# iagostorch/VVC-MIP-GPU

Measured on AMD Instinct MI355X. Metric: 1080p frames/sec, full MIP mode search over all CU sizes; 1/2/4/8 GPU, higher is better.
Workload: dtype int16x2/int32

## Files before the change

vvc-mip-gpu_amd/csrc/mip_kernels.h:

```cpp
#pragma once
#include <hip/hip_runtime.h>
#include <stdint.h>

#include "mipgpu.h"

namespace mipgpu {

struct Job {
  uint32_t cost;
  uint8_t lx, ly;
  uint16_t cu;
};
struct WaveTask {
  uint8_t cls;
  uint8_t ncu;
  uint8_t q0, q1;
  uint32_t cu0;
};

constexpr int kNumClasses = 29;
constexpr int kNumBaseClasses = 17;
constexpr int kClassW[kNumClasses] = {64, 32, 32, 16, 32, 8, 16, 16, 8, 32, 4, 16, 4, 8, 8, 4, 4, 32, 16, 16, 8,
                                      4, 4, 4, 8, 8, 8, 32, 16};
constexpr int kClassH[kNumClasses] = {64, 32, 16, 32, 8, 32, 16, 8, 16, 4, 32, 4, 16, 8, 4, 8, 4, 8, 16, 8, 16,
// ... 25 lines not shown
  uint8_t *best_mode;
  int32_t *best_cost;
  uint32_t *split_acc;
  const uint16_t *dfill;
  const int *dfill_begin;
  int32_t *sad;
  int32_t *satd;
  const WaveTask *tasks;
  const Job *jobs;
  const int *list_begin;
  const uint32_t *fill;
  const int *fill_begin;
  const uint8_t *ctu_var;
  const uint4 *tables;
  int width, height;
  int ctu_cols, nctus;
  int ctu0, nrange;
  int slices;
  uint32_t *queue;
  uint32_t nitems;
  const uint32_t *order;
  uint32_t nframes;
  uint32_t chunks;
  uint64_t *wave_clock;
  uint32_t *status;
  uint32_t *const *frame_status;
  int check_refs;
  uint32_t nonempty;
};
constexpr int kStatusOrig = 0, kStatusRefs = 1, kStatusWords = 4;
constexpr uint32_t kAbove10Bits = 0xfc00fc00u;
constexpr int kClockSlots = 128;
constexpr int kQueueChunks = 8;
constexpr int kQueueWords = 16;
constexpr int kMaxCtuVariants = 255;

constexpr float kAccInitS2 = 0.5f - 1024.0f;
constexpr int kWeightRows = 768, kWeightRowOffS1 = 384, kWeightRowOffS0 = 512;
constexpr int kCtabRows = 384 + 4;
constexpr int kTableBytes = kWeightRows * 16 + kCtabRows * 4;

struct FixupCu {
  uint32_t ctu;
  uint16_t cu;
  uint8_t shape;
  uint8_t pad;
// ... 72 lines not shown
```

vvc-mip-gpu_amd/csrc/mip_search.hip:

```cpp
#include <algorithm>
#include <cstdlib>
#include <type_traits>
#include <utility>

#include <hip/hip_ext.h>

#ifndef MIP_FOUR_WAVE_TWIN
#define MIP_FOUR_WAVE_TWIN 0
#endif
#if MIP_FOUR_WAVE_TWIN
#define launch_search launch_search_four
#define search_resident_groups search_resident_groups_four
#define search_lds_bytes search_lds_bytes_four
#endif

#include "mip_kernels.h"
#include "mip_tables.h"

namespace mipgpu {
namespace {

typedef short __attribute__((ext_vector_type(2))) s2;
typedef unsigned short __attribute__((ext_vector_type(2))) u2;
typedef _Float16 __attribute__((ext_vector_type(2))) h2;
// ... 86 lines not shown
__device__ __forceinline__ void static_for_impl(F &f, std::integer_sequence<int, I...>) {
  (f(std::integral_constant<int, I>{}), ...);
}
template <int N, class F>
__device__ __forceinline__ void static_for(F &&f) {
  static_for_impl(f, std::make_integer_sequence<int, N>{});
}

template <int O>
__device__ __forceinline__ u2 pk_mad_c(u2 a, u2 c) {
  if constexpr (O == 1) {
    return a + c;
  } else {
    u2 d;
    asm("v_pk_mad_u16 %0, %1, %2, %3 op_sel_hi:[1,0,1]" : "=v"(d) : "v"(a), "i"(O), "v"(c));
    return d;
  }
}
template <int O, int C>
__device__ __forceinline__ u2 pk_mad_cc(u2 a) {
  u2 d;
  asm("v_pk_mad_u16 %0, %1, %2, %3 op_sel_hi:[1,0,0]" : "=v"(d) : "v"(a), "i"(O), "i"(C));
  return d;
}

__device__ __forceinline__ void wave_lds_sync() {
  __builtin_amdgcn_fence(__ATOMIC_RELEASE, "wavefront");
  __builtin_amdgcn_wave_barrier();
  __builtin_amdgcn_fence(__ATOMIC_ACQUIRE, "wavefront");
}

template <int W, int H, int VP = kClassV[size_class(W, H)]>
struct Geo {
  static constexpr int SID = class_size_id(W, H);
  static constexpr int R = SID == 2 ? 8 : 4;
  static constexpr int RBS = SID == 0 ? 2 : 4;
  static constexpr int NOUT = R * R;
  static constexpr int UH = W / R, UV = H / R;
  static constexpr int LH = ilog2c(UH), LV = ilog2c(UV);
  static constexpr int S = W / 4;
  static constexpr int V = VP;
  static constexpr int SLOTS = 64 / (S * V);
  static constexpr int KV = R / V;
  static constexpr int CROWS = UH != 1 ? (kSpanChunks && 64 / (S * V) * (R * (R + 1) + 1) > kScratchWords ? R / 2 : R)
                               : 64 / (S * V) * (NOUT + 4) <= kScratchWords ? R
                               : !kSpanChunks ? (SID == 2 ? R / 2 : R)
// ... 721 lines not shown
          emit(std::integral_constant<int, w * G::UV + r>{}, prow);
        });
#pragma unroll
        for (int cc = 0; cc < 4; cc++) prev[cc] = next[cc];
      });
    }
    if constexpr (ORIG::TR) {
      acc.t0 = pair_finish_tr(t0, acc.t0);
      acc.t1 = pair_finish_tr(t1, acc.t1);
    } else {
      acc.t0 = pair_finish(t0, acc.t0);
      acc.t1 = pair_finish(t1, acc.t1);
    }
  }
}

struct Ctx {
  const SearchArgs *a;
  const uint16_t *org;
  const uint16_t *ref;
  const uint8_t *w;
  const uint8_t *zero;
  uint8_t *wave;
  int ctu, frame;
  int fx0, fy0;
};

__device__ __forceinline__ uint32_t floor_sat(float f) { return (uint32_t)f; }

template <int W, int H, int V, bool TR>
__device__ __forceinline__ void phase_a(const Ctx &x, int lane, int ncu, int q, int chunk) {
  using G = Geo<W, H, V>;
  const int r = lane & 15, h = lane >> 4;
  const int m0 = TR ? 2 * q - G::MODES : 2 * q;
  constexpr bool HALF = G::CHUNKED && G::SID != 2;
  constexpr bool TR2 = TR && G::SID == 2 && G::CHUNKED && G::CROWS == 2;
  const int jrow = TR2 ? 8 * (r >> 1) + (r & 1) : (G::SID == 2 && TR) ? 8 * (r >> 2) + (r & 3) : r;
  const uint8_t *abase = x.w + ((G::WBASE + (m0 + (h >> 1)) * G::NOUT + jrow) * 8 + 4 * (h & 1)) * 2;
  const bool bsel = (h >> 1) == (r & 1);
  const uint8_t *bbase = bsel ? x.wave + (r >> 1) * kEntryBytes + 8 * ((h & 1) ^ (TR ? 1 : 0)) : x.zero;
  f4 cin;
  if constexpr (G::SID == 2) {
    cin = *reinterpret_cast<const f4 *>(reinterpret_cast<const float *>(x.w + kWeightRows * 16) + 384);
  } else {
    const float *ct = reinterpret_cast<const float *>(x.w + kWeightRows * 16) + (G::WBASE - kWeightRowOffS1);
    cin = *reinterpret_cast<const f4 *>(ct + (m0 + (r & 1)) * G::NOUT + 4 * h);
  }
  constexpr int NCS = (G::SLOTS + 7) / 8;
// ... 112 lines not shown
#define MIP_PIN_SUMS 1
#endif
__device__ __forceinline__ uint32_t pin_sum(uint32_t v) {
#if MIP_PIN_SUMS
  asm volatile("; pin" : "+v"(v));
#endif
  return v;
}

#ifndef MIP_COST_STORE_AUX
#define MIP_COST_STORE_AUX 0
#endif
struct CtuRows {
  __amdgpu_buffer_rsrc_t r;
  __device__ __forceinline__ explicit CtuRows(int32_t *ctu_block) {
    r = __builtin_amdgcn_make_buffer_rsrc(ctu_block, 0, MIP_COSTS_PER_CTU * 4, 0x00020000);
  }
  __device__ __forceinline__ void store(uint32_t cu_ofs, int mq, int v0, int v1) const {
    typedef unsigned int v2u __attribute__((ext_vector_type(2)));
    __builtin_amdgcn_raw_buffer_store_b64((v2u){(unsigned)v0, (unsigned)v1}, r, (int)cu_ofs, mq * 4, MIP_COST_STORE_AUX);
  }
};

__device__ __forceinline__ int opaque(int v) {
  asm volatile("; opaque" : "+v"(v));
  return v;
}

template <bool TR, bool LAT>
struct ViewOf {
  using type = RefTile<LAT>;
  static __device__ __forceinline__ type make(const RefTile<LAT> &r) { return r; }
};
template <bool LAT>
struct ViewOf<true, LAT> {
  using type = RefTileT<LAT>;
  static __device__ __forceinline__ type make(const RefTile<LAT> &r) { return RefTileT<LAT>{r}; }
};

template <int W, int H, int V, bool LAT, bool DEC, bool TR = false>
__device__ __forceinline__ void run_task(const Ctx &x, const RefTile<LAT> &rt_tile, const WaveTask &task, int lane_in) {
  using G = Geo<W, H, V>;
  const typename ViewOf<TR, LAT>::type rt = ViewOf<TR, LAT>::make(rt_tile);
  const int lane = opaque(lane_in);
  const SearchArgs &a = *x.a;
  const int ncu = task.ncu;
  const Job *jobs = a.jobs + task.cu0;
  const int slot = lane / (G::S * G::V), sub = lane % (G::S * G::V);
  const int v = sub / G::S, sx = sub % G::S, x0 = 4 * sx;
  const bool active = slot < ncu;
  const int cs = min(slot, ncu - 1);
  const Job job = jobs[cs];
  const CuPos c = cu_pos<TR>(job, x.fx0, x.fy0, rt);

  if (lane < ncu) {
    const Job jb = jobs[lane];
    const CuPos cj = cu_pos<TR>(jb, x.fx0, x.fy0, rt);
    write_inputs<W, H>(cj, rt, x.wave + lane * kEntryBytes);
  }
  std::conditional_t<TR, OrigRowsT<H>, OrigRows<H>> orig;
  orig.load(x.org, c.lx + x0, c.ly);
  const size_t ctu_row = ((size_t)x.frame * a.nctus + x.ctu) * MIP_COSTS_PER_CTU;
  const uint32_t cu_ofs = (uint32_t)job.cost * 4;
  const CtuRows rows_cost(a.cost ? a.cost + ctu_row : nullptr), rows_sad(a.sad ? a.sad + ctu_row : nullptr),
      rows_satd(a.satd ? a.satd + ctu_row : nullptr);
  const uint32_t *mine = reinterpret_cast<const uint32_t *>(x.wave + kCuTableBytes) + cs * G::PITCH;
  const Red<G::R, G::RP> red{mine, 0};
  s2 top[4];
  {
    const uint2 tv = rt.top4(c.lx + x0, c.ly - 1);
    const int t4[4] = {(int)(tv.x & 0xffff), (int)(tv.x >> 16), (int)(tv.y & 0xffff), (int)(tv.y >> 16)};
#pragma unroll
    for (int cc = 0; cc < 4; cc++) top[cc] = splat(c.top ? t4[cc] : c.padT);
  }
  constexpr int NLV = (G::R + G::S * G::V - 1) / (G::S * G::V);
  uint32_t lvs[G::PAD && G::CHUNKED ? NLV : 1];
  uint32_t *lcol = reinterpret_cast<uint32_t *>(x.wave + kCuTableBytes) + cs * G::PITCH;
  auto write_left = [&](int chunk) {
#pragma unroll
    for (int j = 0; j < NLV; j++) {
      const int k = sub + j * G::S * G::V;
      if (active && k < G::R && k / G::CROWS == chunk) lcol[(k - chunk * G::CROWS) * G::RP] = lvs[j];
    }
  };
  if constexpr (G::PAD && G::CHUNKED) {
// ... 86 lines not shown
      sad0 = sp & 0xffff, sad1 = sp >> 16, satd0 = tp & 0xffff, satd1 = tp >> 16;
    } else {
      acc.flush();
      sad0 = pin_sum(group_sum<GS>(acc.sad0));
      sad1 = pin_sum(group_sum<GS>(acc.sad1));
      satd0 = pin_sum(group_sum<GS>(acc.satd0));
      satd1 = pin_sum(group_sum<GS>(acc.satd1));
      c0 = min(2 * (int)sad0, (int)satd0);
      c1 = min(2 * (int)sad1, (int)satd1);
    }
    if (active && sub == GS - 1) {
      const int mq = TR ? (2 * q < G::MODES ? 2 * q + G::MODES : 2 * q - G::MODES) : 2 * q;
      if constexpr (DEC) {
        best = min(best, min((uint32_t)c0 << 5 | (uint32_t)mq, (uint32_t)c1 << 5 | (uint32_t)(mq + 1)));
      } else {
        rows_cost.store(cu_ofs, mq, c0, c1);
        if (a.sad) rows_sad.store(cu_ofs, mq, (int)sad0, (int)sad1);
        if (a.satd) rows_satd.store(cu_ofs, mq, (int)satd0, (int)satd1);
      }
    }
  }
  if (DEC && active && sub == G::S * G::V - 1) {
    constexpr int kPairs = G::SID == 2 ? 6 : (G::SID == 1 ? 8 : 16);
    const size_t g = ((size_t)x.frame * a.nctus + x.ctu) * MIP_CUS_PER_CTU + job.cu;
    if (task.q0 == 0 && task.q1 == kPairs) {
      if (a.best_mode) a.best_mode[g] = (uint8_t)(best & 31);
      a.best_cost[g] = (int32_t)(best >> 5);
    } else {
      atomicMin((a.split_acc ? a.split_acc : reinterpret_cast<uint32_t *>(a.best_cost)) + g, best);
    }
  }
}

__device__ __forceinline__ uint2 frame_chunk(const uint16_t *frame, int width, int height, int fx, int fy) {
  const int li = fy * width + fx;
  uint2 v = make_uint2(0, 0);
  if (fy >= 0 && fx >= 0 && li < width * height) v = *reinterpret_cast<const uint2 *>(frame + li);
  return v;
}

template <int P>
struct WindowStager {
  static constexpr int RIT = P / 16;
  static constexpr int NMAIN = (65 + RIT - 1) / RIT;
  static constexpr int NHALO = (65 + P - 1) / P;
  static constexpr int N = NMAIN + NHALO;
  static constexpr uint32_t kOut = 0x80000000u;
// ... 26 lines not shown
      if (k == 0 && top) o = p < 16 ? kOut : o;
    } else {
      o = vhalo + (uint32_t)((k - NMAIN) * P) * W2;
      if (left) o = kOut;
      if (k == NMAIN && top) o = p == 0 ? kOut : o;
    }
    typedef unsigned int v2u __attribute__((ext_vector_type(2)));
    const v2u v = __builtin_amdgcn_raw_buffer_load_b64(rsrc, (int)o, 0, 0);
    return make_uint2(v.x, v.y);
  }
  __device__ __forceinline__ void store(uint16_t *dst, int k, uint2 v) const {
    if (k < NMAIN) {
      v.x += bmx;
      v.y += bmy;
      *reinterpret_cast<uint2 *>(dst + (p / 16 + RIT * k) * kPitch + 4 + 4 * (p & 15)) = v;
    } else {
      v.x += bhx;
      v.y += bhy;
      *reinterpret_cast<uint2 *>(dst + (p + P * (k - NMAIN)) * kPitch) = v;
    }
  }
};

#ifndef MIP_FRAME_STATUS
#define MIP_FRAME_STATUS 1
#endif
__device__ __forceinline__ void flag_above_10_bits(uint32_t bits, const SearchArgs &a, int frame, int word) {
  if (bits & kAbove10Bits) (MIP_FRAME_STATUS && a.frame_status ? a.frame_status[frame] : a.status)[word] = 1u;
}

template <int NT>
__device__ __forceinline__ void stage_tile(uint16_t *dst, const uint16_t *frame, int width, int height,
                                           int x0, int y0, const SearchArgs &a, int fidx) {
  const WindowStager<NT> st(frame, width, height, x0, y0, (int)threadIdx.x);
  constexpr int N = WindowStager<NT>::N;
  uint2 v[N];
#pragma unroll
  for (int k = 0; k < N; k++)
    if (st.valid(k)) v[k] = st.load(k);
  uint32_t bits = 0;
#pragma unroll
  for (int k = 0; k < N; k++)
    if (st.valid(k)) {
      bits |= v[k].x | v[k].y;
      st.store(dst, k, v[k]);
    }
  flag_above_10_bits(bits, a, fidx, kStatusOrig);
}

struct ItemPos {
  int frame, ctu, slice, quad, ctu_x, ctu_y, fx0, fy0;
  __device__ __forceinline__ ItemPos(const SearchArgs &a, uint32_t item) {
    const int per_ctu = 4 * a.slices;
    uint32_t base = item;
    if (a.order) {
      base = a.order[item / a.nframes];
      frame = item % a.nframes;
    } else {
      frame = item / (per_ctu * a.nrange);
    }
    const int gx = base % per_ctu;
    ctu = a.ctu0 + (base / per_ctu) % a.nrange;
    slice = gx % a.slices;
    quad = gx / a.slices;
    ctu_x = 128 * (ctu % a.ctu_cols);
    ctu_y = 128 * (ctu / a.ctu_cols);
    fx0 = ctu_x + 64 * (quad & 1);
    fy0 = ctu_y + 64 * (quad >> 1);
  }
};

template <int NT>
__device__ __forceinline__ void stage_lattice(uint16_t *dst, const uint16_t *frame, int width, int height,
                                              int x0, int y0, bool check, const SearchArgs &a, int fidx) {
  constexpr int kChunks = kPitch / 4, NR = 16 * kChunks, NC = 16 * 65;
  constexpr int NRL = (NR + NT - 1) / NT, NCL = (NC + NT - 1) / NT;
  uint2 rv[NRL];
  uint16_t cv[NCL];
#pragma unroll
  for (int k = 0; k < NRL; k++) {
    const int i = min((int)threadIdx.x + NT * k, NR - 1), row = i / kChunks, ch = i - row * kChunks;
    rv[k] = frame_chunk(frame, width, height, x0 - kColOff + 4 * ch, y0 + 4 * row - 1);
  }
#pragma unroll
  for (int k = 0; k < NCL; k++) {
    const int i = min((int)threadIdx.x + NT * k, NC - 1), col = i / 65, yy = i - col * 65;
    const int fy = y0 + yy - 1, fx = x0 + 4 * col - 1, li = fy * width + fx;
    cv[k] = (fy >= 0 && fx >= 0 && li < width * height) ? frame[li] : 0;
  }
  uint32_t bits = 0;
  const bool exempt_last = width % 128 != 0;
  auto frame_col = [&](int fx) { return fx < width ? fx : fx % width; };
#pragma unroll
  for (int k = 0; k < NRL; k++) {
    const int i = min((int)threadIdx.x + NT * k, NR - 1), row = i / kChunks, ch = i - row * kChunks;
    *reinterpret_cast<uint2 *>(dst + row * kLatRowPitch + 4 * ch) = rv[k];
    if (check) {
      const int fx = x0 - kColOff + 4 * ch;
      const bool skip_y = exempt_last && fx >= 0 && frame_col(fx) == width - 4;
      bits |= rv[k].x | (skip_y ? 0u : rv[k].y);
    }
  }
  uint16_t *cols = dst + 16 * kLatRowPitch;
#pragma unroll
  for (int k = 0; k < NCL; k++) {
    const int i = min((int)threadIdx.x + NT * k, NC - 1), col = i / 65, yy = i - col * 65;
    cols[col * kLatColPitch + yy] = cv[k];
    if (check) {
      const int fx = x0 + 4 * col - 1;
      if (!(exempt_last && fx >= 0 && frame_col(fx) == width - 1)) bits |= cv[k];
    }
  }
  if (check) flag_above_10_bits(bits, a, fidx, kStatusRefs);
}

template <bool ALT, bool PF, int NW = kSearchWaves>
constexpr int kOrgTiles = (PF || NW == kWideWaves) && !ALT ? 2 : 1;
constexpr int kCounterWords = 12;

__device__ __forceinline__ uint32_t queue_chunks(const SearchArgs &a) { return gridDim.x < a.chunks ? gridDim.x : a.chunks; }
__device__ __forceinline__ uint32_t chunk_begin(uint32_t nitems, uint32_t c, uint32_t k) {
  return (uint32_t)((uint64_t)nitems * c / k);
}
__device__ __forceinline__ uint32_t take_item(const SearchArgs &a, uint32_t *empty) {
  const uint32_t k = queue_chunks(a), g = blockIdx.x % k;
  for (uint32_t j = *empty; j < k; j++) {
    const uint32_t c = g + j < k ? g + j : g + j - k;
    const uint32_t b = chunk_begin(a.nitems, c, k), n = chunk_begin(a.nitems, c + 1, k) - b;
    const uint32_t i = atomicAdd(a.queue + c, 1u);
    if (i < n) {
      *empty = j;
      return b + i;
    }
  }
  *empty = k;
  return a.nitems;
}
__device__ __forceinline__ bool far_from_end(const SearchArgs &a, uint32_t item) {
  const uint32_t k = queue_chunks(a), g = blockIdx.x % k;
  const uint32_t b = chunk_begin(a.nitems, g, k), e = chunk_begin(a.nitems, g + 1, k);
  return item >= b && item + 3 * (gridDim.x / k) < e;
}
constexpr uint32_t kTakeItem = 0xffffffffu;

template <bool DEC>
__device__ __forceinline__ void fill_unavailable(const SearchArgs &a, int frame, int ctu, int vq, int slice) {
  if (DEC) {
    const size_t gbase = ((size_t)frame * a.nctus + ctu) * MIP_CUS_PER_CTU;
    const int f0 = a.dfill_begin[vq], nf = a.dfill_begin[vq + 1] - f0;
    for (int i = slice * blockDim.x + threadIdx.x; i < nf; i += a.slices * blockDim.x) {
      const size_t g = gbase + a.dfill[f0 + i];
      if (a.best_mode) a.best_mode[g] = 0xff;
      a.best_cost[g] = kUnavailable;
    }
  } else {
    const size_t cbase = ((size_t)frame * a.nctus + ctu) * (MIP_COSTS_PER_CTU / 4);
    const int f0 = a.fill_begin[vq], nf = a.fill_begin[vq + 1] - f0;
    const uint4 un = make_uint4(kUnavailable, kUnavailable, kUnavailable, kUnavailable);
    for (int i = slice * blockDim.x + threadIdx.x; i < nf; i += a.slices * blockDim.x) {
      const size_t o = cbase + a.fill[f0 + i];
      reinterpret_cast<uint4 *>(a.cost)[o] = un;
      if (a.sad) reinterpret_cast<uint4 *>(a.sad)[o] = un;
      if (a.satd) reinterpret_cast<uint4 *>(a.satd)[o] = un;
    }
  }
}

template <bool ALT, bool DEC>
__device__ __forceinline__ void dispatch_task(const Ctx &x, const RefTile<ALT> &rt, const WaveTask &task, int lane) {
  switch (task.cls) {
#define MIP_CASE(idx, W, H)                                                \
  case idx:                                                                \
    static_assert(kClassW[idx] == W && kClassH[idx] == H, "class table");  \
    if constexpr ((MIP_ONLY_CLASS < 0 || MIP_ONLY_CLASS == idx) && !((MIP_SKIP_CLASSES >> idx) & 1)) \
      run_task<W, H, kClassV[idx], ALT, DEC>(x, rt, task, lane);           \
    break;
    MIP_CASE(0, 64, 64) MIP_CASE(1, 32, 32) MIP_CASE(2, 32, 16) MIP_CASE(3, 16, 32)
    MIP_CASE(4, 32, 8) MIP_CASE(5, 8, 32) MIP_CASE(6, 16, 16) MIP_CASE(7, 16, 8)
    MIP_CASE(8, 8, 16) MIP_CASE(9, 32, 4) MIP_CASE(10, 4, 32) MIP_CASE(11, 16, 4)
// ... 4 lines not shown
#undef MIP_CASE
#define MIP_CASE_TR(idx, W, H)                                                    \
  case idx:                                                                       \
    static_assert(kClassW[idx] == W && kClassH[idx] == H && kClassTR[idx], "class table"); \
    if constexpr ((MIP_ONLY_CLASS < 0 || MIP_ONLY_CLASS == idx) && !((MIP_SKIP_CLASSES >> idx) & 1)) \
      run_task<W, H, kClassV[idx], ALT, DEC, true>(x, rt, task, lane);            \
    break;
    MIP_CASE_TR(21, 4, 32) MIP_CASE_TR(22, 4, 16) MIP_CASE_TR(23, 4, 8) MIP_CASE_TR(24, 8, 32)
    MIP_CASE_TR(25, 8, 16) MIP_CASE_TR(26, 8, 16)
#undef MIP_CASE_TR
    default: break;
  }
}

__device__ __forceinline__ void stamp_item_start(uint64_t *clk) {
  clk[kClockSlots - 3] = __builtin_amdgcn_s_memrealtime();
  clk[kClockSlots - 1] = (uint64_t)__builtin_amdgcn_s_getreg((31 << 11) | 4) |
                         (uint64_t)__builtin_amdgcn_s_getreg((31 << 11) | 20) << 32;
}

template <int NT>
__device__ __forceinline__ void stage_tiles2(uint16_t *dst0, const uint16_t *frame0, int x0, int y0, uint16_t *dst1,
                                             const uint16_t *frame1, int x1, int y1, bool b, int width, int height,
                                             const SearchArgs &a, int f0, int f1) {
  const WindowStager<NT> s0(frame0, width, height, x0, y0, (int)threadIdx.x);
  const WindowStager<NT> s1(frame1, width, height, x1, y1, (int)threadIdx.x);
  constexpr int N = WindowStager<NT>::N;
  uint2 v0[N], v1[N];
#pragma unroll
  for (int k = 0; k < N; k++) {
    if (s0.valid(k)) v0[k] = s0.load(k);
    if (b && s1.valid(k)) v1[k] = s1.load(k);
  }
  uint32_t bits0 = 0, bits1 = 0;
#pragma unroll
  for (int k = 0; k < N; k++) {
    if (s0.valid(k)) {
      bits0 |= v0[k].x | v0[k].y;
      s0.store(dst0, k, v0[k]);
    }
    if (b && s1.valid(k)) {
      bits1 |= v1[k].x | v1[k].y;
      s1.store(dst1, k, v1[k]);
    }
  }
  flag_above_10_bits(bits0, a, f0, kStatusOrig);
  flag_above_10_bits(bits1, a, f1, kStatusOrig);
}

template <bool DEC>
__device__ __forceinline__ void pair_loop(const SearchArgs &a, uint16_t *org_buf, const uint8_t *w, const uint8_t *zero,
                                          uint8_t *waves, uint32_t *counters, int wave, int lane) {
  const uint32_t ne = a.nonempty, npairs = (ne + 1) / 2;
  for (;;) {
    if (threadIdx.x == 0) {
      counters[0] = 0;
      counters[1] = atomicAdd(a.queue, 1u);
    }
    __syncthreads();
    const uint32_t p = counters[1];
    if (p >= npairs) break;
    const uint32_t i0 = p, i1 = ne - 1 - p;
    const bool two = i1 != i0;
    const ItemPos p0(a, i0), p1(a, i1);
    const int vq0 = a.ctu_var[p0.ctu] * 4 + p0.quad, vq1 = a.ctu_var[p1.ctu] * 4 + p1.quad;
    const int l0 = vq0 * a.slices + p0.slice, l1 = vq1 * a.slices + p1.slice;
    const int tb0 = a.list_begin[l0], n0 = a.list_begin[l0 + 1] - tb0;
    const int tb1 = a.list_begin[l1], n1 = two ? a.list_begin[l1 + 1] - tb1 : 0;
    fill_unavailable<DEC>(a, p0.frame, p0.ctu, vq0, p0.slice);
    if (two) fill_unavailable<DEC>(a, p1.frame, p1.ctu, vq1, p1.slice);
    for (uint32_t e = ne + p; e < a.nitems; e += npairs) {
      const ItemPos pe(a, e);
      fill_unavailable<DEC>(a, pe.frame, pe.ctu, a.ctu_var[pe.ctu] * 4 + pe.quad, pe.slice);
    }
    uint16_t *org0 = org_buf, *org1 = org_buf + kTileElems;
    stage_tiles2<64 * kWideWaves>(org0, a.orig + (size_t)p0.frame * a.width * a.height, p0.fx0, p0.fy0, org1,
                                  a.orig + (size_t)p1.frame * a.width * a.height, p1.fx0, p1.fy0, two, a.width,
                                  a.height, a, p0.frame, p1.frame);
    __syncthreads();
    uint64_t *clk0 = a.wave_clock ? a.wave_clock + (size_t)i0 * kClockSlots : nullptr;
    uint64_t *clk1 = a.wave_clock && two ? a.wave_clock + (size_t)i1 * kClockSlots : nullptr;
    if (clk0 && threadIdx.x == 0) {
      stamp_item_start(clk0);
      if (clk1) stamp_item_start(clk1);
    }
    const int m = n0 < n1 ? n0 : n1;
    for (;;) {
      uint32_t tn = 0;
      if (lane == 0) tn = atomicAdd(counters, 1u);
      const int t = (int)__builtin_amdgcn_readfirstlane(tn);
      if (t >= n0 + n1) break;
      const bool second = t < 2 * m ? (t & 1) != 0 : n1 > n0;
      const int k = t < 2 * m ? t >> 1 : t - m;
      const uint64_t c0 = clk0 ? __builtin_readcyclecounter() : 0;
      const WaveTask task = a.tasks[(second ? tb1 : tb0) + k];
      const Ctx x{&a, second ? org1 : org0, second ? org1 : org0, w, zero, waves + wave * kWaveStride,
                  second ? p1.ctu : p0.ctu, second ? p1.frame : p0.frame, second ? p1.fx0 : p0.fx0,
                  second ? p1.fy0 : p0.fy0};
      const RefTile<false> rt{x.ref};
      dispatch_task<false, DEC>(x, rt, task, lane);
      uint64_t *clk = second ? clk1 : clk0;
      if (clk && lane == 0) {
        if (k < kClockSlots - 3) clk[k] = __builtin_readcyclecounter() - c0;
        atomicMax(reinterpret_cast<unsigned long long *>(clk + kClockSlots - 2),
                  (unsigned long long)__builtin_amdgcn_s_memrealtime());
      }
    }
    __syncthreads();
  }
}

#ifndef MIP_WAVES_PER_EU
#define MIP_WAVES_PER_EU (MIP_SIX_WAVES ? 6 : 4)
#endif
#ifndef MIP_TABLES_GLOBAL
#define MIP_TABLES_GLOBAL 0
#endif
constexpr bool kTablesInLds = (!MIP_SIX_WAVES || MIP_SIX_WAVES == 3) && !MIP_TABLES_GLOBAL;
#ifndef MIP_S6_PF
#define MIP_S6_PF 1
#endif
#define MIP_PF_KERNEL (!MIP_SIX_WAVES || (MIP_SIX_WAVES == 3 && MIP_S6_PF))
constexpr bool kPrefetchKernel = MIP_PF_KERNEL;
template <bool ALT, bool DEC, bool PF_, int NW>
__global__ __launch_bounds__(64 * NW, NW == kWideWaves ? 4 : MIP_WAVES_PER_EU) void mip_search_kernel(SearchArgs a) {
  constexpr bool PF = PF_ && !ALT && NW == kSearchWaves && kPrefetchKernel;
  extern __shared__ __attribute__((aligned(16))) uint8_t smem[];
  uint16_t *org_buf = reinterpret_cast<uint16_t *>(smem);
  uint16_t *lattice = org_buf + kOrgTiles<ALT, PF, NW> * kTileElems;
  uint8_t *tab = smem + (kOrgTiles<ALT, PF, NW> * kTileElems + (ALT ? kLatElems : 0)) * 2;
  uint8_t *zero = tab + (kTablesInLds ? kTableBytes : 0);
  uint8_t *waves = zero + kZeroBytes;
  uint32_t *counters = reinterpret_cast<uint32_t *>(waves + NW * kWaveStride);
  const uint8_t *w = kTablesInLds ? tab : reinterpret_cast<const uint8_t *>(a.tables);

  if constexpr (kTablesInLds)
    for (int i = threadIdx.x; i < kTableBytes / 16; i += blockDim.x)
      reinterpret_cast<uint4 *>(tab)[i] = a.tables[i];
  for (int i = threadIdx.x; i < kZeroBytes / 16; i += blockDim.x)
    reinterpret_cast<uint4 *>(zero)[i] = make_uint4(0, 0, 0, 0);
  const int wave = __builtin_amdgcn_readfirstlane(threadIdx.x >> 6), lane = threadIdx.x & 63;

  if (NW == kWideWaves && !ALT && !PF && a.nonempty > 0) {
    pair_loop<DEC>(a, org_buf, w, zero, waves, counters, wave, lane);
  } else {
  if (threadIdx.x < kCounterWords) counters[threadIdx.x] = threadIdx.x == 2 && PF ? kTakeItem : 0u;
  __syncthreads();
  if (!PF) {
    if (threadIdx.x == 0) counters[2] = take_item(a, counters + 8);
    __syncthreads();
  }
  int par = 0;
  for (;;) {
    uint32_t *next_task = counters + 4 * par, *finished = next_task + 1;
    uint32_t item = next_task[2];
    bool staged = PF;
    if (PF && item == kTakeItem) {
      if (threadIdx.x == 0) next_task[3] = take_item(a, counters + 8);
      __syncthreads();
      item = next_task[3];
      staged = false;
    }
    if (item >= a.nitems) break;
    const ItemPos ip(a, item);
    const int ctu = ip.ctu, frame = ip.frame, slice = ip.slice, quad = ip.quad, fx0 = ip.fx0, fy0 = ip.fy0;
    const size_t fofs = (size_t)frame * a.width * a.height;
    const int var = a.ctu_var[ctu];
    const int vq = var * 4 + quad, list = vq * a.slices + slice;
    const int tbase = a.list_begin[list], ntasks = a.list_begin[list + 1] - tbase;
    uint16_t *org = org_buf + (PF ? par * kTileElems : 0);
    uint16_t *ref = ALT ? lattice : org;

    fill_unavailable<DEC>(a, frame, ctu, vq, slice);
    if (ntasks > 0) {
      if (!PF || !staged) {
        stage_tile<64 * NW>(org, a.orig + fofs, a.width, a.height, fx0, fy0, a, frame);
        if (ALT) stage_lattice<64 * NW>(ref, a.refs + fofs, a.width, a.height, fx0, fy0, a.check_refs != 0, a, frame);
        __syncthreads();
      }

      const Ctx x{&a, org, ref, w, zero, waves + wave * kWaveStride, ctu, frame, fx0, fy0};
      const RefTile<ALT> rt{ref};
      uint64_t *clk = a.wave_clock ? a.wave_clock + (size_t)item * kClockSlots : nullptr;
      if (clk && threadIdx.x == 0) stamp_item_start(clk);
      for (;;) {
        uint32_t tn = 0;
        if (lane == 0) tn = atomicAdd(next_task, 1u);
        const int t = (int)__builtin_amdgcn_readfirstlane(tn);
        if (t >= ntasks) break;
#if MIP_PRIO_BALANCE
        {
          const int rem4 = 4 * (ntasks - t);
          if (rem4 > 3 * ntasks) __builtin_amdgcn_s_setprio(3);
          else if (rem4 > 2 * ntasks) __builtin_amdgcn_s_setprio(2);
          else if (rem4 > ntasks) __builtin_amdgcn_s_setprio(1);
          else __builtin_amdgcn_s_setprio(0);
        }
#endif
        const uint64_t c0 = clk ? __builtin_readcyclecounter() : 0;
        const WaveTask task = a.tasks[tbase + t];
        dispatch_task<ALT, DEC>(x, rt, task, lane);
        if (clk && lane == 0 && t < kClockSlots - 3) clk[t] = __builtin_readcyclecounter() - c0;
      }
      if (clk && lane == 0) atomicMax(reinterpret_cast<unsigned long long *>(clk + kClockSlots - 2),
                                      (unsigned long long)__builtin_amdgcn_s_memrealtime());
    }
    if (PF) {
      uint32_t *nxt = counters + 4 * (par ^ 1);
      uint32_t r = 0;
      if (lane == 0) r = atomicAdd(finished, 1u);
      if (__builtin_amdgcn_readfirstlane(r) == 0) {
        uint32_t n = kTakeItem;
        if (lane == 0 && far_from_end(a, item)) n = take_item(a, counters + 8);
        const uint32_t nitem = __builtin_amdgcn_readfirstlane(n);
        if (nitem < a.nitems) {
          const ItemPos np(a, nitem);
          const uint16_t *nframe = a.orig + (size_t)np.frame * a.width * a.height;
          uint16_t *dst = org_buf + (par ^ 1) * kTileElems;
          const WindowStager<64> st(nframe, a.width, a.height, np.fx0, np.fy0, lane);
          constexpr int NL = WindowStager<64>::N, NB = MIP_PF_BATCH;
          uint32_t bits = 0;
#pragma unroll
          for (int k0 = 0; k0 < NL; k0 += NB) {
            uint2 v[NB];
#pragma unroll
            for (int k = 0; k < NB; k++)
              if (k0 + k < NL && st.valid(k0 + k)) v[k] = st.load(k0 + k);
#pragma unroll
            for (int k = 0; k < NB; k++)
              if (k0 + k < NL && st.valid(k0 + k)) {
                bits |= v[k].x | v[k].y;
                st.store(dst, k0 + k, v[k]);
              }
          }
          flag_above_10_bits(bits, a, np.frame, kStatusOrig);
        }
        if (lane == 0) {
          nxt[0] = 0;
          nxt[1] = 0;
          nxt[2] = nitem;
        }
      }
      __syncthreads();
    } else {
      __syncthreads();
      if (threadIdx.x == 0) {
        next_task[0] = 0;
        next_task[2] = take_item(a, counters + 8);
      }
      __syncthreads();
    }
    if (PF) par ^= 1;
  }
  }
  if (threadIdx.x == 0) {
    __threadfence();
    if (atomicAdd(a.queue + kQueueChunks, 1u) == gridDim.x - 1) {
      for (int c = 0; c < kQueueChunks; c++) atomicExch(a.queue + c, 0u);
      atomicExch(a.queue + kQueueChunks, 0u);
    }
  }
}

template <int M>
__device__ __forceinline__ void topk_row(const int32_t *row, int k, uint8_t *mo, int32_t *co) {
  int v[M];
#pragma unroll
  for (int m = 0; m < M; m += 4) {
    const int4 q = *reinterpret_cast<const int4 *>(row + m);
    v[m] = q.x, v[m + 1] = q.y, v[m + 2] = q.z, v[m + 3] = q.w;
  }
  const bool unavailable = v[0] == kUnavailable;
  uint32_t used = 0;
  for (int r = 0; r < k; r++) {
    int best = 0, bc = 0;
    bool found = false;
#pragma unroll
    for (int m = 0; m < M; m++)
      if (!((used >> m) & 1) && (!found || v[m] < bc)) best = m, bc = v[m], found = true;
    const bool ok = found && !unavailable;
    if (ok) used |= 1u << best;
    if (mo) mo[r] = ok ? (uint8_t)best : 0xff;
// ... 87 lines not shown
                             resident_per_cu<false, false, true, S>(), resident_per_cu<false, true, true, S>()
#endif
                             });
  return per_cu >= 1 ? cus * per_cu : 0;
}

hipError_t launch_search(const SearchArgs &args, int nframes, bool alt_refs, int resident, bool wide, hipStream_t s,
                         hipEvent_t done) {
  if (args.slices < 1 || !args.queue || !args.status || resident < 1) return hipErrorInvalidValue;
  SearchArgs a = args;
  if (a.ctu0 < 0 || a.nrange < 1 || a.ctu0 + a.nrange > a.nctus) return hipErrorInvalidValue;
  const long long nitems = (long long)(4 * a.slices) * a.nrange * nframes;
  if (nitems >= 0xffffffffLL) return hipErrorInvalidValue;
  a.nitems = (uint32_t)nitems;
  const char *qc = getenv("MIPGPU_QUEUE_CHUNKS");
  a.chunks = qc && atoi(qc) >= 1 && atoi(qc) <= kQueueChunks
                 ? (uint32_t)atoi(qc)
                 : (a.nitems >= (uint32_t)MIP_PREFETCH_MIN_ITEMS * (uint32_t)resident ? (uint32_t)kQueueChunks : 1u);
  a.nframes = (uint32_t)nframes;
  if (a.chunks > 1 || a.ctu0 != 0 || a.nrange != a.nctus) a.order = nullptr;
  if (!wide || alt_refs || !a.order || a.chunks != 1 || a.nonempty > a.nitems) a.nonempty = 0;
  const char *env = getenv("MIPGPU_GROUPS");
  const int groups = std::min<long long>(env && atoi(env) > 0 ? atoi(env) : resident, a.nitems);
  const bool dec = a.cost == nullptr;
  if (dec && (!a.best_cost || !a.dfill_begin)) return hipErrorInvalidValue;
  const bool pf = kPrefetchKernel && !alt_refs && !wide && a.nitems >= (uint32_t)MIP_PREFETCH_MIN_ITEMS * (uint32_t)groups;
  const size_t lds = search_lds_bytes(alt_refs, pf, wide ? kWideWaves : kSearchWaves);
  const dim3 grid(groups);
  constexpr int S = kSearchWaves, L = kWideWaves;
  (void)L;
  auto go = [&](auto kern, const dim3 &block) {
    if (done) hipExtLaunchKernelGGL(kern, grid, block, (uint32_t)lds, s, nullptr, done, 0u, a);
    else hipLaunchKernelGGL(kern, grid, block, lds, s, a);
  };
  if (wide) {
#if MIP_FOUR_WAVE_TWIN
    return hipErrorInvalidValue;
#else
    const dim3 block(64 * L);
    if (alt_refs) {
      if (dec) go(mip_search_kernel<true, true, false, L>, block);
      else go(mip_search_kernel<true, false, false, L>, block);
    } else {
      if (dec) go(mip_search_kernel<false, true, false, L>, block);
      else go(mip_search_kernel<false, false, false, L>, block);
    }
// ... 37 lines not shown
```

Baseline: 7879.

## Decode work items once per block and precompute queue chunk bounds on host

Wave 0 now decodes each dequeued item (frame, CTU, task list range, flattened frame-CTU index) and publishes it to an LDS record. Other waves read it with readfirstlane instead of each recomputing ItemPos and reloading list_begin and ctu_var. Chunk boundaries, the chunk count and the tail threshold are precomputed on the host, replacing 64-bit division in take_item and far_from_end. Kernel arguments are re-read through an opaque kernarg pointer so the compiler does not keep them live in SGPRs across the task loop. The aim is lower scalar register pressure and less per-item integer work, at the cost of extra LDS traffic and more complex item handoff.

After: 7878. Within noise of the previous version (-0.0%).

```diff
diff --git a/vvc-mip-gpu_amd/csrc/mip_kernels.h b/vvc-mip-gpu_amd/csrc/mip_kernels.h
--- a/vvc-mip-gpu_amd/csrc/mip_kernels.h
+++ b/vvc-mip-gpu_amd/csrc/mip_kernels.h
@@ -71,6 +71,8 @@
   const uint32_t *order;
   uint32_t nframes;
   uint32_t chunks;
+  uint32_t qchunks, chunk_q, chunk_r, chunk_rcp;
+  uint32_t tail_items;
   uint64_t *wave_clock;
   uint32_t *status;
   uint32_t *const *frame_status;
diff --git a/vvc-mip-gpu_amd/csrc/mip_search.hip b/vvc-mip-gpu_amd/csrc/mip_search.hip
--- a/vvc-mip-gpu_amd/csrc/mip_search.hip
+++ b/vvc-mip-gpu_amd/csrc/mip_search.hip
@@ -132,6 +132,11 @@
   u2 d;
   asm("v_pk_mad_u16 %0, %1, %2, %3 op_sel_hi:[1,0,0]" : "=v"(d) : "v"(a), "i"(O), "i"(C));
   return d;
+}
+
+__device__ __forceinline__ int opaque(int v) {
+  asm volatile("; opaque" : "+v"(v));
+  return v;
 }
 
 __device__ __forceinline__ void wave_lds_sync() {
@@ -899,8 +904,8 @@
   const uint8_t *w;
   const uint8_t *zero;
   uint8_t *wave;
-  int ctu, frame;
   int fx0, fy0;
+  uint32_t fctu;
 };
 
 __device__ __forceinline__ uint32_t floor_sat(float f) { return (uint32_t)f; }
@@ -1059,11 +1064,6 @@
   }
 };
 
-__device__ __forceinline__ int opaque(int v) {
-  asm volatile("; opaque" : "+v"(v));
-  return v;
-}
-
 template <bool TR, bool LAT>
 struct ViewOf {
   using type = RefTile<LAT>;
@@ -1097,7 +1097,7 @@
   }
   std::conditional_t<TR, OrigRowsT<H>, OrigRows<H>> orig;
   orig.load(x.org, c.lx + x0, c.ly);
-  const size_t ctu_row = ((size_t)x.frame * a.nctus + x.ctu) * MIP_COSTS_PER_CTU;
+  const size_t ctu_row = (size_t)x.fctu * MIP_COSTS_PER_CTU;
   const uint32_t cu_ofs = (uint32_t)job.cost * 4;
   const CtuRows rows_cost(a.cost ? a.cost + ctu_row : nullptr), rows_sad(a.sad ? a.sad + ctu_row : nullptr),
       rows_satd(a.satd ? a.satd + ctu_row : nullptr);
@@ -1230,7 +1230,7 @@
   }
   if (DEC && active && sub == G::S * G::V - 1) {
     constexpr int kPairs = G::SID == 2 ? 6 : (G::SID == 1 ? 8 : 16);
-    const size_t g = ((size_t)x.frame * a.nctus + x.ctu) * MIP_CUS_PER_CTU + job.cu;
+    const size_t g = (size_t)x.fctu * MIP_CUS_PER_CTU + job.cu;
     if (task.q0 == 0 && task.q1 == kPairs) {
       if (a.best_mode) a.best_mode[g] = (uint8_t)(best & 31);
       a.best_cost[g] = (int32_t)(best >> 5);
@@ -1303,17 +1303,27 @@
   }
 };
 
+__device__ __forceinline__ const SearchArgs &item_args() {
+  typedef const __attribute__((address_space(4))) SearchArgs *KernargPtr;
+  KernargPtr p = (KernargPtr)__builtin_amdgcn_kernarg_segment_ptr();
+  asm volatile("; item args" : "+s"(p));
+  return *(const SearchArgs *)p;
+}
+
 #ifndef MIP_FRAME_STATUS
 #define MIP_FRAME_STATUS 1
 #endif
-__device__ __forceinline__ void flag_above_10_bits(uint32_t bits, const SearchArgs &a, int frame, int word) {
-  if (bits & kAbove10Bits) (MIP_FRAME_STATUS && a.frame_status ? a.frame_status[frame] : a.status)[word] = 1u;
+__device__ __forceinline__ void flag_above_10_bits(uint32_t bits, int frame, int word) {
+  if (bits & kAbove10Bits) {
+    const SearchArgs &a = item_args();
+    (MIP_FRAME_STATUS && a.frame_status ? a.frame_status[frame] : a.status)[word] = 1u;
+  }
 }
 
 template <int NT>
 __device__ __forceinline__ void stage_tile(uint16_t *dst, const uint16_t *frame, int width, int height,
-                                           int x0, int y0, const SearchArgs &a, int fidx) {
-  const WindowStager<NT> st(frame, width, height, x0, y0, (int)threadIdx.x);
+                                           int x0, int y0, int fidx) {
+  const WindowStager<NT> st(frame, width, height, x0, y0, opaque((int)threadIdx.x));
   constexpr int N = WindowStager<NT>::N;
   uint2 v[N];
 #pragma unroll
@@ -1326,7 +1336,7 @@
       bits |= v[k].x | v[k].y;
       st.store(dst, k, v[k]);
     }
-  flag_above_10_bits(bits, a, fidx, kStatusOrig);
+  flag_above_10_bits(bits, fidx, kStatusOrig);
 }
 
 struct ItemPos {
@@ -1351,21 +1361,53 @@
   }
 };
 
+struct Item {
+  int frame, fx0, fy0;
+  int vq, slice;
+  int tbase, ntasks;
+  uint32_t fctu;
+};
+constexpr int kItemWords = 8;
+__device__ __forceinline__ Item decode_item(const SearchArgs &a, uint32_t item) {
+  const ItemPos p(a, item);
+  Item it;
+  it.frame = p.frame, it.fx0 = p.fx0, it.fy0 = p.fy0, it.slice = p.slice;
+  it.vq = a.ctu_var[p.ctu] * 4 + p.quad;
+  const int list = it.vq * a.slices + p.slice;
+  it.tbase = a.list_begin[list];
+  it.ntasks = a.list_begin[list + 1] - it.tbase;
+  it.fctu = (uint32_t)p.frame * (uint32_t)a.nctus + (uint32_t)p.ctu;
+  return it;
+}
+__device__ __forceinline__ void publish_item(uint32_t *rec, const Item &it) {
+  reinterpret_cast<uint4 *>(rec)[0] = make_uint4((uint32_t)it.frame, (uint32_t)it.fx0, (uint32_t)it.fy0, it.fctu);
+  reinterpret_cast<uint4 *>(rec)[1] = make_uint4((uint32_t)it.vq, (uint32_t)it.slice, (uint32_t)it.tbase, (uint32_t)it.ntasks);
+}
+__device__ __forceinline__ Item read_item(const uint32_t *rec) {
+  const uint4 r0 = reinterpret_cast<const uint4 *>(rec)[0], r1 = reinterpret_cast<const uint4 *>(rec)[1];
+  auto u = [](uint32_t v) { return (int)__builtin_amdgcn_readfirstlane(v); };
+  Item it;
+  it.frame = u(r0.x), it.fx0 = u(r0.y), it.fy0 = u(r0.z), it.fctu = (uint32_t)u(r0.w);
+  it.vq = u(r1.x), it.slice = u(r1.y), it.tbase = u(r1.z), it.ntasks = u(r1.w);
+  return it;
+}
+
 template <int NT>
 __device__ __forceinline__ void stage_lattice(uint16_t *dst, const uint16_t *frame, int width, int height,
-                                              int x0, int y0, bool check, const SearchArgs &a, int fidx) {
+                                              int x0, int y0, bool check, int fidx) {
+  const int tid = opaque((int)threadIdx.x);
   constexpr int kChunks = kPitch / 4, NR = 16 * kChunks, NC = 16 * 65;
   constexpr int NRL = (NR + NT - 1) / NT, NCL = (NC + NT - 1) / NT;
   uint2 rv[NRL];
   uint16_t cv[NCL];
 #pragma unroll
   for (int k = 0; k < NRL; k++) {
-    const int i = min((int)threadIdx.x + NT * k, NR - 1), row = i / kChunks, ch = i - row * kChunks;
+    const int i = min(tid + NT * k, NR - 1), row = i / kChunks, ch = i - row * kChunks;
     rv[k] = frame_chunk(frame, width, height, x0 - kColOff + 4 * ch, y0 + 4 * row - 1);
   }
 #pragma unroll
   for (int k = 0; k < NCL; k++) {
-    const int i = min((int)threadIdx.x + NT * k, NC - 1), col = i / 65, yy = i - col * 65;
+    const int i = min(tid + NT * k, NC - 1), col = i / 65, yy = i - col * 65;
     const int fy = y0 + yy - 1, fx = x0 + 4 * col - 1, li = fy * width + fx;
     cv[k] = (fy >= 0 && fx >= 0 && li < width * height) ? frame[li] : 0;
   }
@@ -1374,7 +1416,7 @@
   auto frame_col = [&](int fx) { return fx < width ? fx : fx % width; };
 #pragma unroll
   for (int k = 0; k < NRL; k++) {
-    const int i = min((int)threadIdx.x + NT * k, NR - 1), row = i / kChunks, ch = i - row * kChunks;
+    const int i = min(tid + NT * k, NR - 1), row = i / kChunks, ch = i - row * kChunks;
     *reinterpret_cast<uint2 *>(dst + row * kLatRowPitch + 4 * ch) = rv[k];
     if (check) {
       const int fx = x0 - kColOff + 4 * ch;
@@ -1385,29 +1427,30 @@
   uint16_t *cols = dst + 16 * kLatRowPitch;
 #pragma unroll
   for (int k = 0; k < NCL; k++) {
-    const int i = min((int)threadIdx.x + NT * k, NC - 1), col = i / 65, yy = i - col * 65;
+    const int i = min(tid + NT * k, NC - 1), col = i / 65, yy = i - col * 65;
     cols[col * kLatColPitch + yy] = cv[k];
     if (check) {
       const int fx = x0 + 4 * col - 1;
       if (!(exempt_last && fx >= 0 && frame_col(fx) == width - 1)) bits |= cv[k];
     }
   }
-  if (check) flag_above_10_bits(bits, a, fidx, kStatusRefs);
+  if (check) flag_above_10_bits(bits, fidx, kStatusRefs);
 }
 
 template <bool ALT, bool PF, int NW = kSearchWaves>
 constexpr int kOrgTiles = (PF || NW == kWideWaves) && !ALT ? 2 : 1;
-constexpr int kCounterWords = 12;
-
-__device__ __forceinline__ uint32_t queue_chunks(const SearchArgs &a) { return gridDim.x < a.chunks ? gridDim.x : a.chunks; }
-__device__ __forceinline__ uint32_t chunk_begin(uint32_t nitems, uint32_t c, uint32_t k) {
-  return (uint32_t)((uint64_t)nitems * c / k);
+constexpr int kItemRecord = 12;
+constexpr int kCounterWords = kItemRecord + 2 * 8;
+
+
+__device__ __forceinline__ uint32_t chunk_begin(const SearchArgs &a, uint32_t c) {
+  return a.chunk_q * c + (a.chunk_r * c * a.chunk_rcp >> 16);
 }
 __device__ __forceinline__ uint32_t take_item(const SearchArgs &a, uint32_t *empty) {
-  const uint32_t k = queue_chunks(a), g = blockIdx.x % k;
+  const uint32_t k = a.qchunks, g = empty[1];
   for (uint32_t j = *empty; j < k; j++) {
     const uint32_t c = g + j < k ? g + j : g + j - k;
-    const uint32_t b = chunk_begin(a.nitems, c, k), n = chunk_begin(a.nitems, c + 1, k) - b;
+    const uint32_t b = chunk_begin(a, c), n = chunk_begin(a, c + 1) - b;
     const uint32_t i = atomicAdd(a.queue + c, 1u);
     if (i < n) {
       *empty = j;
@@ -1417,17 +1460,28 @@
   *empty = k;
   return a.nitems;
 }
-__device__ __forceinline__ bool far_from_end(const SearchArgs &a, uint32_t item) {
-  const uint32_t k = queue_chunks(a), g = blockIdx.x % k;
-  const uint32_t b = chunk_begin(a.nitems, g, k), e = chunk_begin(a.nitems, g + 1, k);
-  return item >= b && item + 3 * (gridDim.x / k) < e;
+__device__ __forceinline__ bool far_from_end(const SearchArgs &a, uint32_t item, const uint32_t *empty) {
+  const uint32_t g = empty[1];
+  const uint32_t b = chunk_begin(a, g), e = chunk_begin(a, g + 1);
+  return item >= b && item + a.tail_items < e;
 }
 constexpr uint32_t kTakeItem = 0xffffffffu;
+__device__ __forceinline__ uint32_t take_decoded(uint32_t *empty, uint32_t *rec, int lane) {
+  const SearchArgs &a = item_args();
+  uint32_t n = 0;
+  if (lane == 0) n = take_item(a, empty);
+  const uint32_t item = __builtin_amdgcn_readfirstlane(n);
+  if (item < a.nitems) {
+    const Item it = decode_item(a, item);
+    if (lane == 0) publish_item(rec, it);
+  }
+  return item;
+}
 
 template <bool DEC>
-__device__ __forceinline__ void fill_unavailable(const SearchArgs &a, int frame, int ctu, int vq, int slice) {
+__device__ __forceinline__ void fill_unavailable(const SearchArgs &a, uint32_t fctu, int vq, int slice) {
   if (DEC) {
-    const size_t gbase = ((size_t)frame * a.nctus + ctu) * MIP_CUS_PER_CTU;
+    const size_t gbase = (size_t)fctu * MIP_CUS_PER_CTU;
     const int f0 = a.dfill_begin[vq], nf = a.dfill_begin[vq + 1] - f0;
     for (int i = slice * blockDim.x + threadIdx.x; i < nf; i += a.slices * blockDim.x) {
       const size_t g = gbase + a.dfill[f0 + i];
@@ -1435,7 +1489,7 @@
       a.best_cost[g] = kUnavailable;
     }
   } else {
-    const size_t cbase = ((size_t)frame * a.nctus + ctu) * (MIP_COSTS_PER_CTU / 4);
+    const size_t cbase = (size_t)fctu * (MIP_COSTS_PER_CTU / 4);
     const int f0 = a.fill_begin[vq], nf = a.fill_begin[vq + 1] - f0;
     const uint4 un = make_uint4(kUnavailable, kUnavailable, kUnavailable, kUnavailable);
     for (int i = slice * blockDim.x + threadIdx.x; i < nf; i += a.slices * blockDim.x) {
@@ -1486,9 +1540,10 @@
 template <int NT>
 __device__ __forceinline__ void stage_tiles2(uint16_t *dst0, const uint16_t *frame0, int x0, int y0, uint16_t *dst1,
                                              const uint16_t *frame1, int x1, int y1, bool b, int width, int height,
-                                             const SearchArgs &a, int f0, int f1) {
-  const WindowStager<NT> s0(frame0, width, height, x0, y0, (int)threadIdx.x);
-  const WindowStager<NT> s1(frame1, width, height, x1, y1, (int)threadIdx.x);
+                                             int f0, int f1) {
+  const int tid = opaque((int)threadIdx.x);
+  const WindowStager<NT> s0(frame0, width, height, x0, y0, tid);
+  const WindowStager<NT> s1(frame1, width, height, x1, y1, tid);
   constexpr int N = WindowStager<NT>::N;
   uint2 v0[N], v1[N];
 #pragma unroll
@@ -1508,42 +1563,58 @@
       s1.store(dst1, k, v1[k]);
     }
   }
-  flag_above_10_bits(bits0, a, f0, kStatusOrig);
-  flag_above_10_bits(bits1, a, f1, kStatusOrig);
+  flag_above_10_bits(bits0, f0, kStatusOrig);
+  flag_above_10_bits(bits1, f1, kStatusOrig);
 }
 
 template <bool DEC>
 __device__ __forceinline__ void pair_loop(const SearchArgs &a, uint16_t *org_buf, const uint8_t *w, const uint8_t *zero,
                                           uint8_t *waves, uint32_t *counters, int wave, int lane) {
-  const uint32_t ne = a.nonempty, npairs = (ne + 1) / 2;
+  const uint32_t ne = item_args().nonempty, npairs = (ne + 1) / 2;
+  uint32_t *rec0 = counters + kItemRecord, *rec1 = rec0 + kItemWords;
   for (;;) {
-    if (threadIdx.x == 0) {
-      counters[0] = 0;
-      counters[1] = atomicAdd(a.queue, 1u);
+    if (wave == 0) {
+      const SearchArgs &da = item_args();
+      uint32_t pn = 0;
+      if (lane == 0) pn = atomicAdd(da.queue, 1u);
+      const uint32_t pw = __builtin_amdgcn_readfirstlane(pn);
+      if (pw < npairs) {
+        const Item d0 = decode_item(da, pw);
+        Item d1 = d0;
+        if (ne - 1 - pw != pw) d1 = decode_item(da, ne - 1 - pw);
+        else d1.ntasks = 0;
+        if (lane == 0) {
+          publish_item(rec0, d0);
+          publish_item(rec1, d1);
+        }
+      }
+      if (lane == 0) {
+        counters[0] = 0;
+        counters[1] = pw;
+      }
     }
     __syncthreads();
     const uint32_t p = counters[1];
     if (p >= npairs) break;
     const uint32_t i0 = p, i1 = ne - 1 - p;
     const bool two = i1 != i0;
-    const ItemPos p0(a, i0), p1(a, i1);
-    const int vq0 = a.ctu_var[p0.ctu] * 4 + p0.quad, vq1 = a.ctu_var[p1.ctu] * 4 + p1.quad;
-    const int l0 = vq0 * a.slices + p0.slice, l1 = vq1 * a.slices + p1.slice;
-    const int tb0 = a.list_begin[l0], n0 = a.list_begin[l0 + 1] - tb0;
-    const int tb1 = a.list_begin[l1], n1 = two ? a.list_begin[l1 + 1] - tb1 : 0;
-    fill_unavailable<DEC>(a, p0.frame, p0.ctu, vq0, p0.slice);
-    if (two) fill_unavailable<DEC>(a, p1.frame, p1.ctu, vq1, p1.slice);
-    for (uint32_t e = ne + p; e < a.nitems; e += npairs) {
-      const ItemPos pe(a, e);
-      fill_unavailable<DEC>(a, pe.frame, pe.ctu, a.ctu_var[pe.ctu] * 4 + pe.quad, pe.slice);
+    const Item p0 = read_item(rec0), p1 = read_item(rec1);
+    const int tb0 = p0.tbase, n0 = p0.ntasks, tb1 = p1.tbase, n1 = p1.ntasks;
+    const SearchArgs &ia = item_args();
+    fill_unavailable<DEC>(ia, p0.fctu, p0.vq, p0.slice);
+    if (two) fill_unavailable<DEC>(ia, p1.fctu, p1.vq, p1.slice);
+    for (uint32_t e = ne + p; e < ia.nitems; e += npairs) {
+      const Item pe = decode_item(ia, e);
+      fill_unavailable<DEC>(ia, pe.fctu, pe.vq, pe.slice);
     }
     uint16_t *org0 = org_buf, *org1 = org_buf + kTileElems;
-    stage_tiles2<64 * kWideWaves>(org0, a.orig + (size_t)p0.frame * a.width * a.height, p0.fx0, p0.fy0, org1,
-                                  a.orig + (size_t)p1.frame * a.width * a.height, p1.fx0, p1.fy0, two, a.width,
-                                  a.height, a, p0.frame, p1.frame);
+    stage_tiles2<64 * kWideWaves>(org0, ia.orig + (size_t)p0.frame * ia.width * ia.height, p0.fx0, p0.fy0, org1,
+                                  ia.orig + (size_t)p1.frame * ia.width * ia.height, p1.fx0, p1.fy0, two, ia.width,
+                                  ia.height, p0.frame, p1.frame);
     __syncthreads();
-    uint64_t *clk0 = a.wave_clock ? a.wave_clock + (size_t)i0 * kClockSlots : nullptr;
-    uint64_t *clk1 = a.wave_clock && two ? a.wave_clock + (size_t)i1 * kClockSlots : nullptr;
+    uint64_t *const wclk = ia.wave_clock;
+    uint64_t *clk0 = wclk ? wclk + (size_t)i0 * kClockSlots : nullptr;
+    uint64_t *clk1 = wclk && two ? wclk + (size_t)i1 * kClockSlots : nullptr;
     if (clk0 && threadIdx.x == 0) {
       stamp_item_start(clk0);
       if (clk1) stamp_item_start(clk1);
@@ -1559,8 +1630,7 @@
       const uint64_t c0 = clk0 ? __builtin_readcyclecounter() : 0;
       const WaveTask task = a.tasks[(second ? tb1 : tb0) + k];
       const Ctx x{&a, second ? org1 : org0, second ? org1 : org0, w, zero, waves + wave * kWaveStride,
-                  second ? p1.ctu : p0.ctu, second ? p1.frame : p0.frame, second ? p1.fx0 : p0.fx0,
-                  second ? p1.fy0 : p0.fy0};
+                  second ? p1.fx0 : p0.fx0, second ? p1.fy0 : p0.fy0, second ? p1.fctu : p0.fctu};
       const RefTile<false> rt{x.ref};
       dispatch_task<false, DEC>(x, rt, task, lane);
       uint64_t *clk = second ? clk1 : clk0;
@@ -1605,47 +1675,55 @@
     reinterpret_cast<uint4 *>(zero)[i] = make_uint4(0, 0, 0, 0);
   const int wave = __builtin_amdgcn_readfirstlane(threadIdx.x >> 6), lane = threadIdx.x & 63;
 
-  if (NW == kWideWaves && !ALT && !PF && a.nonempty > 0) {
+  if (NW == kWideWaves && !ALT && !PF && item_args().nonempty > 0) {
     pair_loop<DEC>(a, org_buf, w, zero, waves, counters, wave, lane);
   } else {
-  if (threadIdx.x < kCounterWords) counters[threadIdx.x] = threadIdx.x == 2 && PF ? kTakeItem : 0u;
+  if (threadIdx.x < kCounterWords)
+    counters[threadIdx.x] = threadIdx.x == 2 && PF ? kTakeItem : (threadIdx.x == 9 ? blockIdx.x % item_args().qchunks : 0u);
   __syncthreads();
   if (!PF) {
-    if (threadIdx.x == 0) counters[2] = take_item(a, counters + 8);
+    if (wave == 0) {
+      const uint32_t first = take_decoded(counters + 8, counters + kItemRecord, lane);
+      if (lane == 0) counters[2] = first;
+    }
     __syncthreads();
   }
   int par = 0;
   for (;;) {
     uint32_t *next_task = counters + 4 * par, *finished = next_task + 1;
+    uint32_t *item_rec = counters + kItemRecord + (PF ? par * kItemWords : 0);
     uint32_t item = next_task[2];
     bool staged = PF;
     if (PF && item == kTakeItem) {
-      if (threadIdx.x == 0) next_task[3] = take_item(a, counters + 8);
+      if (wave == 0) {
+        const uint32_t late = take_decoded(counters + 8, item_rec, lane);
+        if (lane == 0) next_task[3] = late;
+      }
       __syncthreads();
       item = next_task[3];
       staged = false;
     }
-    if (item >= a.nitems) break;
-    const ItemPos ip(a, item);
-    const int ctu = ip.ctu, frame = ip.frame, slice = ip.slice, quad = ip.quad, fx0 = ip.fx0, fy0 = ip.fy0;
-    const size_t fofs = (size_t)frame * a.width * a.height;
-    const int var = a.ctu_var[ctu];
-    const int vq = var * 4 + quad, list = vq * a.slices + slice;
-    const int tbase = a.list_begin[list], ntasks = a.list_begin[list + 1] - tbase;
+    const SearchArgs &ia = item_args();
+    if (item >= ia.nitems) break;
+    const Item it = read_item(item_rec);
+    const int frame = it.frame, fx0 = it.fx0, fy0 = it.fy0;
+    const int tbase = it.tbase, ntasks = it.ntasks;
     uint16_t *org = org_buf + (PF ? par * kTileElems : 0);
     uint16_t *ref = ALT ? lattice : org;
 
-    fill_unavailable<DEC>(a, frame, ctu, vq, slice);
+    fill_unavailable<DEC>(ia, it.fctu, it.vq, it.slice);
     if (ntasks > 0) {
       if (!PF || !staged) {
-        stage_tile<64 * NW>(org, a.orig + fofs, a.width, a.height, fx0, fy0, a, frame);
-        if (ALT) stage_lattice<64 * NW>(ref, a.refs + fofs, a.width, a.height, fx0, fy0, a.check_refs != 0, a, frame);
+        const size_t fofs = (size_t)frame * ia.width * ia.height;
+        stage_tile<64 * NW>(org, ia.orig + fofs, ia.width, ia.height, fx0, fy0, frame);
+        if (ALT) stage_lattice<64 * NW>(ref, ia.refs + fofs, ia.width, ia.height, fx0, fy0, ia.check_refs != 0, frame);
         __syncthreads();
       }
 
-      const Ctx x{&a, org, ref, w, zero, waves + wave * kWaveStride, ctu, frame, fx0, fy0};
+      const Ctx x{&a, org, ref, w, zero, waves + wave * kWaveStride, fx0, fy0, it.fctu};
       const RefTile<ALT> rt{ref};
-      uint64_t *clk = a.wave_clock ? a.wave_clock + (size_t)item * kClockSlots : nullptr;
+      uint64_t *const wclk = ia.wave_clock;
+      uint64_t *clk = wclk ? wclk + (size_t)item * kClockSlots : nullptr;
       if (clk && threadIdx.x == 0) stamp_item_start(clk);
       for (;;) {
         uint32_t tn = 0;
@@ -1674,14 +1752,16 @@
       uint32_t r = 0;
       if (lane == 0) r = atomicAdd(finished, 1u);
       if (__builtin_amdgcn_readfirstlane(r) == 0) {
+        const SearchArgs &na = item_args();
         uint32_t n = kTakeItem;
-        if (lane == 0 && far_from_end(a, item)) n = take_item(a, counters + 8);
+        if (lane == 0 && far_from_end(na, item, counters + 8)) n = take_item(na, counters + 8);
         const uint32_t nitem = __builtin_amdgcn_readfirstlane(n);
-        if (nitem < a.nitems) {
-          const ItemPos np(a, nitem);
-          const uint16_t *nframe = a.orig + (size_t)np.frame * a.width * a.height;
+        if (nitem < na.nitems) {
+          const Item np = decode_item(na, nitem);
+          if (lane == 0) publish_item(counters + kItemRecord + (par ^ 1) * kItemWords, np);
+          const uint16_t *nframe = na.orig + (size_t)np.frame * na.width * na.height;
           uint16_t *dst = org_buf + (par ^ 1) * kTileElems;
-          const WindowStager<64> st(nframe, a.width, a.height, np.fx0, np.fy0, lane);
+          const WindowStager<64> st(nframe, na.width, na.height, np.fx0, np.fy0, opaque(lane));
           constexpr int NL = WindowStager<64>::N, NB = MIP_PF_BATCH;
           uint32_t bits = 0;
 #pragma unroll
@@ -1697,7 +1777,7 @@
                 st.store(dst, k0 + k, v[k]);
               }
           }
-          flag_above_10_bits(bits, a, np.frame, kStatusOrig);
+          flag_above_10_bits(bits, np.frame, kStatusOrig);
         }
         if (lane == 0) {
           nxt[0] = 0;
@@ -1708,9 +1788,10 @@
       __syncthreads();
     } else {
       __syncthreads();
-      if (threadIdx.x == 0) {
-        next_task[0] = 0;
-        next_task[2] = take_item(a, counters + 8);
+      if (threadIdx.x == 0) next_task[0] = 0;
+      if (wave == 0) {
+        const uint32_t next = take_decoded(counters + 8, item_rec, lane);
+        if (lane == 0) next_task[2] = next;
       }
       __syncthreads();
     }
@@ -1719,9 +1800,10 @@
   }
   if (threadIdx.x == 0) {
     __threadfence();
-    if (atomicAdd(a.queue + kQueueChunks, 1u) == gridDim.x - 1) {
-      for (int c = 0; c < kQueueChunks; c++) atomicExch(a.queue + c, 0u);
-      atomicExch(a.queue + kQueueChunks, 0u);
+    uint32_t *queue = item_args().queue;
+    if (atomicAdd(queue + kQueueChunks, 1u) == gridDim.x - 1) {
+      for (int c = 0; c < kQueueChunks; c++) atomicExch(queue + c, 0u);
+      atomicExch(queue + kQueueChunks, 0u);
     }
   }
 }
@@ -1855,6 +1937,12 @@
   if (!wide || alt_refs || !a.order || a.chunks != 1 || a.nonempty > a.nitems) a.nonempty = 0;
   const char *env = getenv("MIPGPU_GROUPS");
   const int groups = std::min<long long>(env && atoi(env) > 0 ? atoi(env) : resident, a.nitems);
+  if (groups < 1) return hipErrorInvalidValue;
+  a.qchunks = std::min<uint32_t>(a.chunks, (uint32_t)groups);
+  a.chunk_q = a.nitems / a.qchunks;
+  a.chunk_r = a.nitems % a.qchunks;
+  a.chunk_rcp = (65536u + a.qchunks - 1) / a.qchunks;
+  a.tail_items = 3u * ((uint32_t)groups / a.qchunks);
   const bool dec = a.cost == nullptr;
   if (dec && (!a.best_cost || !a.dfill_begin)) return hipErrorInvalidValue;
   const bool pf = kPrefetchKernel && !alt_refs && !wide && a.nitems >= (uint32_t)MIP_PREFETCH_MIN_ITEMS * (uint32_t)groups;
```
